# stratosphere/rdfind

Hardware: AMD Instinct MI355X
Metric: CIND-discovery triples/sec (higher is better)
Workload: dtype u32

## Files before the change

rdfind_amd/_lib.py:

```python
from __future__ import annotations

import ctypes
import os

import numpy as np

from . import codes

_HERE = os.path.dirname(os.path.abspath(__file__))
LIB_PATH = os.environ.get("RDFIND_HIP_LIB") or os.path.join(_HERE, "librdfind_hip.so")

RDF_CLEAN_IMPLIED = 1
RDF_STRATEGY_ALL_AT_ONCE = 2
RDF_SHARD_LOCAL_SLICE = 4
RDF_USE_ASSOCIATION_RULES = 8

EXPORTED_SYMBOLS = (
    "rdf_ctx_create", "rdf_ctx_destroy", "rdf_last_error", "rdf_version", "rdf_set_triples",
    "rdf_set_triples_device", "rdf_frequent_conditions", "rdf_build_capture_groups", "rdf_discover_cinds",
    "rdf_run", "rdf_cind_count", "rdf_copy_cinds", "rdf_decode_capture", "rdf_binary_key_count",
    "rdf_copy_binary_keys", "rdf_stage_times", "rdf_kernel_times", "rdf_sync",
    "rdf_copy_cinds_range", "rdf_cind_checksum", "rdf_last_stats", "rdf_shard_begin", "rdf_shard_step",
    "rdf_shard_export", "rdf_shard_import", "rdf_set_dictionary", "rdf_format_size", "rdf_format_cinds",
    "rdf_distinct_triples", "rdf_copy_triples", "rdf_parse_ntriples", "rdf_copy_terms",
# ... 3 lines not shown
    "rdf_discover_cinds_paged", "rdf_next_page", "rdf_shard_parse_begin", "rdf_shard_dictionary_begin", "rdf_num_terms",
    "rdf_dictionary_terms", "rdf_copy_result_refs", "rdf_release_scratch", "rdf_set_handover",
    "rdf_copy_result_refs_async", "rdf_handover_wait", "rdf_set_result_form", "rdf_heavy_chunk_count",
    "rdf_copy_result_heavy", "rdf_parse_begin", "rdf_parse_chunk", "rdf_parse_end", "rdf_copy_term_heap",
    "rdf_rewrite_terms", "rdf_condition_histogram", "rdf_join_histogram", "rdf_copy_histogram", "rdf_count_literals",
    "rdf_cind_stats_begin", "rdf_cind_stats_add", "rdf_cind_stats_end", "rdf_cind_histogram", "rdf_copy_top_refs",
    "rdf_select_cinds", "rdf_selected_count", "rdf_copy_selected_decoded", "rdf_format_selected_size",
    "rdf_format_selected", "rdf_find_terms", "rdf_check_cinds", "rdf_copy_check_rows", "rdf_copy_check_examples",
)
RDF_CHK_ABSENT = 0xFFFFFFFE
RDF_CHK_MAX_EXAMPLES = 16
RDF_SEL_ANY = 0xFFFFFFFF
RDF_SEL_MAX_PATTERNS = 256
RDF_SEL_COUNT_ONLY = 1
SEL_CODES = (10, 12, 14, 17, 20, 21, 33, 34, 35)
SEL_ALL_CODES = 0x1FF
RDF_CS_SHAPE, RDF_CS_SUPPORT, RDF_CS_REFS, RDF_CS_INDEGREE = 1, 2, 3, 4
RDF_JH_NO_FIS = 1
RDF_RW_ASCIIFY = 1
RDF_NT_TABS = 1

TEST_SYMBOLS = ("rdf_test_scan", "rdf_test_scan_batch", "rdf_test_radix", "rdf_test_radix_passes",
                "rdf_test_radix_segments", "rdf_test_paths", "rdf_test_rewrite_form", "rdf_test_cind_stats_times",
                "rdf_test_fc_trace", "rdf_test_fc_report", "rdf_test_copy_frequent_unary", "rdf_test_unary_lookup")
REWRITE_FORMS = {0: None, 1: "lds", 2: "global"}
SCAN_U32_U32, SCAN_U32_U64, SCAN_U64_U64 = range(3)
SCAN_DTYPES = {SCAN_U32_U32: (np.uint32, np.uint32), SCAN_U32_U64: (np.uint32, np.uint64),
               SCAN_U64_U64: (np.uint64, np.uint64)}
RADIX_SORT_BITS, RADIX_SORT_DROP, RADIX_PART_HASHED, RADIX_PART_U32 = range(4)
K1_FORMS = {0: None, 1: "partitioned", 2: "radix", 3: "atomic"}
K2_FORMS = {0: None, 1: "plain", 2: "split", 3: "radix", 4: "atomic"}
K3_FORMS = {0: None, 1: "onepass", 2: "twopass"}

X_DONE, X_ALLREDUCE_SUM_U32, X_ALLREDUCE_SUM_U64, X_ALLREDUCE_MIN_U64, X_ALLGATHERV_U64, X_ALLTOALLV_U64 = range(6)
MAX_RANKS = 64

TIMER_NAMES = ("unary", "binary", "emit", "sort", "support", "groups", "heavymask", "pivot", "light", "esort",
               "hcount", "rules", "hwrite", "class", "cemit")


class FcStats(ctypes.Structure):
    _fields_ = [("min_support", ctypes.c_uint32), ("n_ar_suppressed", ctypes.c_uint32),
                ("n_frequent_unary", ctypes.c_uint64 * 3), ("n_binary_keys", ctypes.c_uint64),
                ("n_frequent_binary", ctypes.c_uint64)]


class ParseStats(ctypes.Structure):
# ... 200 lines not shown
        "rdf_dictionary_terms": (i32, [P, P, u64, P, u64, P]),
        "rdf_discover_cinds_paged": (i32, [P, u32, u64, ctypes.POINTER(CindStats)]),
        "rdf_next_page": (i32, [P, ctypes.POINTER(u32), ctypes.POINTER(u64), ctypes.POINTER(u64)]),
        "rdf_host_free": (None, [P]),
        "rdf_shard_begin": (i32, [P, u32, u32, u32, ctypes.c_char_p, u32]),
        "rdf_shard_step": (i32, [P, ctypes.POINTER(Exchange)]),
        "rdf_shard_export": (i32, [P, P]),
        "rdf_shard_import": (i32, [P, P, u64]),
        "rdf_test_scan": (i32, [P, ctypes.c_int, P, u64, u32, u32, ctypes.c_int, ctypes.c_int, P, ctypes.POINTER(u64),
                                ctypes.POINTER(u32)]),
        "rdf_test_scan_batch": (i32, [P, ctypes.c_int, P, u64, u32, P, ctypes.POINTER(u32)]),
        "rdf_test_radix": (i32, [P, ctypes.c_int, P, u64, ctypes.c_int, ctypes.c_int, u64, P, ctypes.POINTER(u64),
                                 ctypes.POINTER(u32)]),
        "rdf_test_radix_passes": (ctypes.c_int, [ctypes.c_int]),
        "rdf_test_radix_segments": (i32, [P, P, u64, P, u64, P, u32, ctypes.c_int, ctypes.c_int, ctypes.c_int32, u32, u32,
                                          P, ctypes.POINTER(u64), ctypes.POINTER(u32)]),
        "rdf_test_paths": (i32, [P, ctypes.POINTER(PathReport)]),
        "rdf_test_rewrite_form": (i32, [P, ctypes.POINTER(u32)]),
        "rdf_test_cind_stats_times": (i32, [P, ctypes.POINTER(ctypes.c_float)]),
        "rdf_test_fc_trace": (i32, [P, ctypes.c_int]),
        "rdf_test_fc_report": (i32, [P, ctypes.POINTER(FcReport)]),
        "rdf_test_copy_frequent_unary": (i32, [P, P, u64, ctypes.POINTER(u64), ctypes.POINTER(u64)]),
        "rdf_test_unary_lookup": (i32, [P, P, u64, P, P, ctypes.POINTER(u32)]),
    }
    for name, (res, args) in sig.items():
        fn = getattr(lib, name, None) if name in TEST_SYMBOLS else getattr(lib, name)
        if fn is None:
            continue
        fn.restype = res
        fn.argtypes = args
    _lib = lib
    return lib


class PinnedBuffer:

    def __init__(self, count: int, dtype):
        self.lib = load()
        self.nbytes = max(int(count), 1) * np.dtype(dtype).itemsize
        self.ptr = self.lib.rdf_host_alloc(self.nbytes)
        if not self.ptr:
            raise RdfError(f"rdf_host_alloc({self.nbytes}) failed")
        self.array = np.ctypeslib.as_array((ctypes.c_uint8 * self.nbytes).from_address(self.ptr)).view(dtype)

    def __del__(self):
        if getattr(self, "ptr", None):
# ... 414 lines not shown
        out = np.empty_like(a)
        n_out, ok = ctypes.c_uint64(), ctypes.c_uint32()
        rc = self._test_fn("rdf_test_radix")(self.ptr, op, a.ctypes.data, a.shape[0], lo, hi, hmask, out.ctypes.data,
                                     ctypes.byref(n_out), ctypes.byref(ok))
        self.test_canaries_ok = bool(ok.value)
        self._check(rc, "rdf_test_radix")
        return out[: n_out.value], bool(ok.value)

    def test_radix_segments(self, src, counts, bases=None, stride=0, w0=0, bits=64, bump=None):
        a = np.ascontiguousarray(src, dtype=np.uint64)
        cnt = np.ascontiguousarray(counts, dtype=np.uint64)
        base = None if bases is None else np.ascontiguousarray(bases, dtype=np.uint64)
        assert base is None or base.shape == cnt.shape
        out = np.empty(max(int(cnt.sum()), 1), np.uint64)
        bseg, bdig, bdelta = bump if bump else (0, 0, 0)
        n_out, ok = ctypes.c_uint64(), ctypes.c_uint32()
        rc = self._test_fn("rdf_test_radix_segments")(
            self.ptr, a.ctypes.data, a.shape[0], None if base is None else base.ctypes.data, stride, cnt.ctypes.data,
            cnt.shape[0], w0, bits, bdelta, bseg, bdig, out.ctypes.data, ctypes.byref(n_out), ctypes.byref(ok))
        self.test_canaries_ok = bool(ok.value)
        self._check(rc, "rdf_test_radix_segments")
        return out[: n_out.value], bool(ok.value)

    def test_paths(self) -> dict:
        r = PathReport()
        self._check(self._test_fn("rdf_test_paths")(self.ptr, ctypes.byref(r)), "rdf_test_paths")
        d = _struct_dict(r)
        d["k1_form"], d["k2_form"], d["k3_form"] = K1_FORMS[r.k1_form], K2_FORMS[r.k2_form], K3_FORMS[r.k3_form]
        for name in ("dense_on", "light_stage", "light_hiocc", "light_ordered", "light_side", "light_two_pass", "sig_on",
                     "piv2_on", "k3_hist"):
            d[name] = bool(d[name])
        return d

    def test_fc_trace(self, on: bool = True):
        self._check(self._test_fn("rdf_test_fc_trace")(self.ptr, int(on)), "rdf_test_fc_trace")

    def test_fc_report(self) -> dict:
        r = FcReport()
        self._check(self._test_fn("rdf_test_fc_report")(self.ptr, ctypes.byref(r)), "rdf_test_fc_report")
        d = _struct_dict(r)
        d["k1_form"], d["k2_form"], d["traced"] = K1_FORMS[r.k1_form], K2_FORMS[r.k2_form], bool(r.traced)
        return d

    def test_copy_frequent_unary(self):
        U, n3 = ctypes.c_uint64(), (ctypes.c_uint64 * 3)()
        fn = self._test_fn("rdf_test_copy_frequent_unary")
# ... 257 lines not shown
```

rdfind_amd/csrc/rdfind_hip.hip:

```cpp
#include <algorithm>
#include <cstdio>
#include <cstring>
#include <cstdlib>
#include <string>
#include <chrono>
#include <vector>
#include <utility>
#include <initializer_list>
#include <unordered_map>

#include "../../include/rdfind_hip.h"
#include "test_abi.h"
#include "primitives.hpp"
#include "radix_host.hpp"
#include "kernels.inl"
#include "switches.hpp"

using namespace rdf;

#define RDF_VERSION "rdfind_amd 0.1 (gfx950)"

#define RDF_CTX_BUFFERS(B) \
     \
    B(INPUT, scal) \
// ... 38 lines not shown
     \
     \
     \
     \
     \
    B(RUN, chk_rows) B(RUN, chk_ex) B(RUN, chk_cand) B(RUN, chk_keys) B(RUN, chk_keys_tmp) B(RUN, chk_flag) B(RUN, chk_pos) \
    B(RUN, chk_ucap) B(RUN, chk_side) B(RUN, chk_cnt) B(RUN, chk_inb) B(RUN, chk_tab) B(RUN, chk_w) B(RUN, chk_woff) \
    B(RUN, chk_rec) B(RUN, chk_rec_tmp) B(RUN, chk_qval) B(RUN, chk_qoff) B(RUN, chk_nit) B(RUN, chk_ioff) \
    B(RUN, chk_viol) B(RUN, chk_vpre) B(RUN, chk_scal) \
     \
    B(RUN, frank) B(RUN, fval) B(RUN, fext) \
    B(RUN, cnt) B(SPARE_FC, tkeys) B(RUN, tcnt) B(RUN, bkeys) B(RUN, bkeys_tmp) B(RUN, lkeys) B(RUN, lvals) B(RUN, flags) \
    B(RUN, pos) \
     \
    B(RUN, uhist) B(SPARE_FC, urecs) B(RUN, usl) B(RUN, cntg) B(RUN, fstage) B(RUN, bfreq) B(RUN, boff) B(RUN, fbits) \
    B(SPARE_FC, brkeys) \
     \
    B(SPARE_FC, brkeys2) B(RUN, bstart2) \
     \
     \
    B(RUN, arcnt) B(RUN, ar_bits) B(RUN, ar_rules) B(RUN, arref) \
     \
    B(SPARE_GROUPS, rec) B(SPARE_GROUPS, rec_tmp) B(RUN, support) B(RUN, fidx) B(RUN, fcap) B(RUN, info) \
    B(SPARE_GROUPS, fk) B(SPARE_GROUPS, fk_tmp) B(RUN, fpos) B(RUN, cstart) B(RUN, skip) B(RUN, gflag) B(RUN, gexcl) \
    B(RUN, goff) B(RUN, gcap) B(RUN, gmap) B(RUN, csup) B(RUN, doff) B(RUN, dcur) B(RUN, dgrp) \
    B(RUN, hist) B(RUN, heavy_list) B(RUN, hbit) B(RUN, bcomp) B(RUN, bkeyc) B(RUN, pcnt) B(RUN, poff) B(RUN, pcur) \
    B(RUN, plist) \
     \
     \
    B(RUN, jhist) B(RUN, rsup) B(RUN, offp) B(RUN, jbh) B(RUN, lsup) \
     \
     \
     \
    B(SPARE_GROUPS, rstore) B(RUN, jrmap) B(RUN, ecache) \
     \
    B(RUN, ukey) B(RUN, utab) B(RUN, urep) B(RUN, ucnt) B(RUN, unoff) B(RUN, uebin) B(RUN, umem) \
     \
    B(RUN, hot) B(RUN, hotc) \
     \
    B(RUN, pivot) B(RUN, nchl) B(RUN, nchh) B(RUN, choffl) B(RUN, choffh) B(RUN, epairs) B(RUN, epairs_tmp) B(RUN, eoff) \
    B(RUN, hcounts) B(RUN, hoff) B(RUN, hbits) B(RUN, cbits) B(RUN, hown) B(RUN, cown) B(RUN, sbase) B(RUN, dcls) \
    B(RUN, crep) B(RUN, out) B(RUN, stage_rows) \
     \
    B(INPUT, dheap) B(INPUT, dtoff) B(RUN, cslen) B(RUN, csoff) B(RUN, cstr) B(RUN, flen) B(RUN, floff) B(RUN, fbuf) \
     \
    B(RUN, drows) B(RUN, ppart) \
     \
// ... 1974 lines not shown
    tend(c, RDF_T_EMIT);
    u64 Je = 0;
    if (n && !onepass) {
        TRY(read_u64(c, overflow, &c->hscal[8]));
        if (c->hscal[8])
            return fail(c, RDF_ERR_LIMIT, "K3: a block emitted more records than its scanned region (records past it "
                                          "were not written)");
    }
    if (reuse) {
        Je = c->ecache_je[slot];
    } else {
        if (je_early == ~0ull) {
            TRY(read_scalars(c, onepass ? 4 : 1));
            je_early = c->hscal[0];
            if (onepass && n && c->hscal[3] >= je_early) c->J_emit += c->hscal[3] - je_early;
        }
        Je = je_early;
        if (cache > 0) c->ecache_je[slot] = Je;
    }
    if (Je > slot_cap) return fail(c, RDF_ERR_LIMIT, "K3 emitted more records than the join range was sized for");
    return g_sort_support(c, ebuf, c->rec_tmp.as<u64>(), Je, sup, Jout, nullptr);
}

static rdf_status g_fresh_bounds(rdf_ctx* c, const u64* keys, u64 J) {
    hipStream_t st = c->stream;
    HIP_TRY(c, hipMemsetAsync(c->cstart.p, 0xff, (c->ncap + 1) * 4, st));
    hipLaunchKernelGGL(k_fresh_bounds, dim3(grid_for(J + 1, RDF_BLOCK, kGrid)), dim3(RDF_BLOCK), 0, st, keys, J, c->ncap,
                       c->joinbits, c->flags.as<u32>(), c->cstart.as<u32>());
    hipLaunchKernelGGL(k_cstart_fix, dim3(grid_for(c->ncap + 1, RDF_BLOCK, kGrid)), dim3(RDF_BLOCK), 0, st, keys, J, c->ncap,
                       c->joinbits, c->cstart.as<u32>());
    return RDF_OK;
}

static rdf_status g_sort_support(rdf_ctx* c, u64* keys, u64* tmp, u64 Je, u32* sup, u64* Jout, u64* keep_out) {
    hipStream_t st = c->stream;
    const int capbits = c->capbits, joinbits = c->joinbits;
    c->J_emit += Je;
    u64 J = 0;
    tbegin(c, RDF_T_SORT);
    HIP_TRY(c, radix_sort_u64_drop(c->ws, keys, tmp, Je, capbits + joinbits, (u32*)dscal(c, 1), &J, st));
    if (keep_out && keys != keep_out) {
        if (J) HIP_TRY(c, hipMemcpyAsync(keep_out, keys, J * 8, hipMemcpyDeviceToDevice, st));
        keys = keep_out;
    }
    tend(c, RDF_T_SORT);
    c->sort_passes_records += Je + (u64)(radix_sort_passes(capbits + joinbits) - 1) * J;
    return g_support_sorted(c, keys, J, sup, Jout);
}

static rdf_status g_support_sorted(rdf_ctx* c, u64* keys, u64 J, u32* sup, u64* Jout) {
    hipStream_t st = c->stream;
    const u64 ncap = c->ncap;
    *Jout = J;
    c->rec_sorted = keys;
    ENSURE(c, flags, std::max<u64>(J, 1) * 4);
    ENSURE(c, fpos, (J + 1) * 4);
    ENSURE(c, cstart, (ncap + 1) * 4);
    tbegin(c, RDF_T_SUPPORT);
    TRY(g_fresh_bounds(c, keys, J));
    HIP_TRY(c, exclusive_scan_u32(c->ws, c->flags.as<u32>(), c->fpos.as<u32>(), J, c->fpos.as<u32>() + J, st));
    if (ncap)
        hipLaunchKernelGGL(k_run_support, dim3(grid_for(ncap, RDF_BLOCK, kGrid)), dim3(RDF_BLOCK), 0, st, c->cstart.as<u32>(),
                           ncap, c->fpos.as<u32>(), sup);
    tend(c, RDF_T_SUPPORT);
    return RDF_OK;
}

static rdf_status g_emit_sort_support(rdf_ctx* c, int proj) {
    TRY(g_record_bits(c));
    HIP_TRY(c, hipEventRecord(c->ev[2], c->stream));
    c->J_emit = 0;
    c->sort_passes_records = 0;
    ENSURE(c, support, std::max<u64>(c->ncap, 1) * 4);
    u64 J = 0;
    TRY(g_emit_range(c, proj, shard_sel(c), 9 * c->n, c->support.as<u32>(), &J));
    c->J = J;
    return RDF_OK;
}

static rdf_status g_compact_captures(rdf_ctx* c) {
    hipStream_t st = c->stream;
    const u32 V = c->V ? c->V : 1;
    const u64 ncap = c->ncap;
    ENSURE(c, flags, std::max<u64>(ncap, 1) * 4);
    ENSURE(c, fidx, (ncap + 1) * 4);
    hipLaunchKernelGGL(k_support_flags, dim3(grid_for(ncap, RDF_BLOCK, kGrid)), dim3(RDF_BLOCK), 0, st,
                       c->support.as<u32>(), ncap, c->ms, c->flags.as<u32>());
    HIP_TRY(c, exclusive_scan_u32(c->ws, c->flags.as<u32>(), c->fidx.as<u32>(), ncap, c->fidx.as<u32>() + ncap, st));
    u32 C = 0, Cu = 0;
    {
        u64 v[2];
        TRY(read_multi(c, {{c->fidx.as<u32>() + ncap, 4}, {c->fidx.as<u32>() + 2ull * c->U, 4}}, v));
        C = (u32)v[0];
        Cu = (u32)v[1];
    }
    c->C = C;
    c->Cu = Cu;
    ENSURE(c, fcap, std::max<u64>(C, 1) * 4);
    ENSURE(c, info, std::max<u64>(C, 1) * sizeof(CapInfo));
    hipLaunchKernelGGL(k_compact_captures, dim3(grid_for(ncap, RDF_BLOCK, kGrid)), dim3(RDF_BLOCK), 0, st,
                       c->support.as<u32>(), c->fidx.as<u32>(), ncap, c->ms, c->fcap.as<u32>(), c->info.as<CapInfo>());
    ENSURE(c, fext, std::max<u64>(C, 1) * 4);
    if (C)
        hipLaunchKernelGGL(k_external_ids, dim3(grid_for(C, RDF_BLOCK, kGrid)), dim3(RDF_BLOCK), 0, st, c->fcap.as<u32>(), C,
                           2u * c->U, V, c->fval.as<u32>(), c->Us, c->Up, c->fext.as<u32>());
    return RDF_OK;
}

static rdf_status g_compact_groups(rdf_ctx* c) {
    hipStream_t st = c->stream;
    const u32 V = c->V ? c->V : 1;
    const u64 ncap = c->ncap, J = c->J;
    const int joinbits = c->joinbits;
    u64* keys = c->rec_sorted;
    tbegin(c, RDF_T_SUPPORT);
    ENSURE(c, flags, std::max(J, ncap) * 4);
    TRY(g_compact_captures(c));
    const u32 C = c->C;
    ENSURE(c, skip, (ncap + 1) * 4);
    if (ncap)
        hipLaunchKernelGGL(k_skip_counts, dim3(grid_for(ncap, RDF_BLOCK, kGrid)), dim3(RDF_BLOCK), 0, st, c->cstart.as<u32>(),
                           c->fpos.as<u32>(), c->support.as<u32>(), ncap, c->ms, c->flags.as<u32>());
    HIP_TRY(c, exclusive_scan_u32(c->ws, c->flags.as<u32>(), c->skip.as<u32>(), ncap, c->skip.as<u32>() + ncap, st));
    u64 fs[2];
    TRY(read_multi(c, {{c->fpos.as<u32>() + J, 4}, {c->skip.as<u32>() + ncap, 4}}, fs));
    const u64 Jf = fs[0] - fs[1];
    c->Jf = Jf;
    u64* dk = keys == c->rec.as<u64>() ? c->rec_tmp.as<u64>() : c->rec.as<u64>();
    ENSURE(c, fk, std::max<u64>(Jf, 1) * 8);
    ENSURE(c, fk_tmp, std::max<u64>(Jf, 1) * 8);
    if (J)
        hipLaunchKernelGGL(k_keep_scatter, dim3(grid_for(J, RDF_BLOCK, kGrid)), dim3(RDF_BLOCK), 0, st, keys, J, joinbits,
                           c->fpos.as<u32>(), c->skip.as<u32>(), c->support.as<u32>(), c->ms, c->fidx.as<u32>(), dk,
                           c->fk.as<u64>());
    tend(c, RDF_T_SUPPORT);
    tbegin(c, RDF_T_GROUPS);
    ENSURE(c, csup, std::max<u64>(C, 1) * 4);
    ENSURE(c, doff, (C + 1ull) * 8);
    ENSURE(c, dgrp, std::max<u64>(Jf, 1) * 4);
    if (C)
        hipLaunchKernelGGL(k_info_support_u32, dim3(grid_for(C, RDF_BLOCK, kGrid)), dim3(RDF_BLOCK), 0, st,
                           c->info.as<CapInfo>(), C, c->csup.as<u32>());
    if (Jf) {
        hipLaunchKernelGGL(k_key_offsets, dim3(grid_for(C + 1ull, RDF_BLOCK, kGrid)), dim3(RDF_BLOCK), 0, st, dk, Jf, C,
                           c->doff.as<u64>());
        u64* tk = c->fk.as<u64>();
        u64* tt = c->fk_tmp.as<u64>();
        HIP_TRY(c, radix_sort_u64_bits(c->ws, tk, tt, Jf, 32, 32 + joinbits, st));
        if (tk != c->fk.as<u64>()) std::swap(c->fk, c->fk_tmp);
    } else {
        HIP_TRY(c, hipMemsetAsync(c->doff.p, 0, (C + 1ull) * 8, st));
    }
    ENSURE(c, gflag, std::max<u64>(Jf, 1) * 4);
    ENSURE(c, gexcl, (Jf + 1) * 4);
    if (Jf)
        hipLaunchKernelGGL(k_group_flags, dim3(grid_for(Jf, RDF_BLOCK, kGrid)), dim3(RDF_BLOCK), 0, st, c->fk.as<u64>(), Jf,
                           c->gflag.as<u32>());
    HIP_TRY(c, exclusive_scan_u32(c->ws, c->gflag.as<u32>(), c->gexcl.as<u32>(), Jf, c->gexcl.as<u32>() + Jf, st));
    u32 G32 = 0;
    TRY(read_u32(c, c->gexcl.as<u32>() + Jf, &G32));
    const u64 G = G32;
    c->G = G;
    ENSURE(c, goff, (G + 1) * 8);
    ENSURE(c, gcap, std::max<u64>(Jf, 1) * 4 + 16);
    ENSURE(c, gmap, (u64)V * 4);
    if (Jf) {
        hipLaunchKernelGGL(k_group_build, dim3(grid_for(Jf, RDF_BLOCK, kGrid)), dim3(RDF_BLOCK), 0, st, c->fk.as<u64>(), Jf,
                           c->gflag.as<u32>(), c->gexcl.as<u32>(), c->goff.as<u64>(), c->gcap.as<u32>(), c->gmap.as<u32>());
        hipLaunchKernelGGL(k_dgrp, dim3(grid_for(Jf, RDF_BLOCK, kGrid)), dim3(RDF_BLOCK), 0, st, dk, Jf, c->gmap.as<u32>(),
                           c->dgrp.as<u32>());
    }
    c->hscal[14] = Jf;
    HIP_TRY(c, hipMemcpyAsync(c->goff.as<u64>() + G, c->hscal + 14, 8, hipMemcpyHostToDevice, st));
    tend(c, RDF_T_GROUPS);
    return RDF_OK;
}

static rdf_status g_range_keep_plan(rdf_ctx* c) {
    const std::vector<rdf_ctx::JoinRange>& ranges = c->jranges;
    c->jr_keep = false;
    if (!c->sw.range_keep || ranges.empty() || ranges.size() > EMIT_MAX_RANGES) return RDF_OK;
    u64 total = 0;
    c->jr_seg.assign(ranges.size() + 1, 0);
    c->jr_J.assign(ranges.size(), 0);
    for (size_t k = 0; k < ranges.size(); ++k) {
        c->jr_seg[k] = total;
        total += ranges[k].recs;
    }
    c->jr_seg[ranges.size()] = total;
    size_t free_b = 0, total_b = 0;
    if (hipMemGetInfo(&free_b, &total_b) != hipSuccess) return RDF_OK;
// ... 130 lines not shown
    for (size_t k = 0; k < ranges.size(); ++k) {
        const rdf_ctx::JoinRange& r = ranges[k];
        u64 J = 0;
        JoinSel js = own;
        js.lo = r.lo;
        js.hi = r.hi;
        if (c->jr_keep) {
            u64* seg = c->rstore.as<u64>() + c->jr_seg[k];
            TRY(g_sort_support(c, seg, c->rec.as<u64>(), c->jr_seg[k + 1] - c->jr_seg[k], c->rsup.as<u32>(), &J, seg));
            c->jr_J[k] = J;
        } else {
            TRY(g_emit_range(c, proj, js, cap_rec, c->rsup.as<u32>(), &J, 1 + (int)k));
        }
        Jtot += J;
        if (ncap)
            hipLaunchKernelGGL(k_add_u32, dim3(grid_for(ncap, RDF_BLOCK, kGrid)), dim3(RDF_BLOCK), 0, st, c->support.as<u32>(),
                               c->rsup.as<u32>(), ncap);
    }
    c->J = Jtot;
    return RDF_OK;
}

static rdf_status g_restore_range(rdf_ctx* c, size_t k, u64* Jout) {
    hipStream_t st = c->stream;
    const u64 J = c->jr_J[k], ncap = c->ncap;
    u64* keys = c->rstore.as<u64>() + c->jr_seg[k];
    ENSURE(c, flags, std::max<u64>(J, 1) * 4);
    ENSURE(c, fpos, (J + 1) * 4);
    ENSURE(c, cstart, (ncap + 1) * 4);
    ENSURE(c, rec, std::max<u64>(c->jr_cap_rec, 1) * 8);
    tbegin(c, RDF_T_SUPPORT);
    TRY(g_fresh_bounds(c, keys, J));
    HIP_TRY(c, exclusive_scan_u32(c->ws, c->flags.as<u32>(), c->fpos.as<u32>(), J, c->fpos.as<u32>() + J, st));
    tend(c, RDF_T_SUPPORT);
    c->rec_sorted = keys;
    *Jout = J;
    return RDF_OK;
}

static rdf_status g_ranges_groups(rdf_ctx* c, int proj, JoinSel own, const u32* local_sup) {
    hipStream_t st = c->stream;
    const u32 V = c->V ? c->V : 1;
    const u64 ncap = c->ncap;
    const int joinbits = c->joinbits;
    const std::vector<rdf_ctx::JoinRange>& ranges = c->jranges;
    const u64 cap_rec = c->jr_cap_rec;
    const u64 J_emit = c->J_emit, Jtot = c->J;
    tbegin(c, RDF_T_SUPPORT);
    TRY(g_compact_captures(c));
    const u32 C = c->C;
    ENSURE(c, csup, std::max<u64>(C, 1) * 4);
    ENSURE(c, doff, (C + 1ull) * 8);
    ENSURE(c, dcur, std::max<u64>(C, 1) * 4);
    if (C)
        hipLaunchKernelGGL(k_info_support_u32, dim3(grid_for(C, RDF_BLOCK, kGrid)), dim3(RDF_BLOCK), 0, st,
                           c->info.as<CapInfo>(), C, c->csup.as<u32>());
// ... 8 lines not shown
    tend(c, RDF_T_SUPPORT);
    u64 Jf = 0;
    TRY(read_u64(c, c->doff.as<u64>() + C, &Jf));
    c->Jf = Jf;
    const u64 Gmax = std::min<u64>(V, Jf);
    ENSURE(c, goff, (Gmax + 1) * 8);
    ENSURE(c, gcap, std::max<u64>(Jf, 1) * 4 + 16);
    ENSURE(c, gmap, (u64)V * 4);
    ENSURE(c, dgrp, std::max<u64>(Jf, 1) * 4);
    ENSURE(c, offp, (C + 1ull) * 8);
    ENSURE(c, skip, (ncap + 1) * 4);
    HIP_TRY(c, hipMemsetAsync(c->dcur.p, 0, std::max<u64>(C, 1) * 4, st));
    u64 Jf0 = 0, G0 = 0;
    for (size_t k = 0; k < ranges.size(); ++k) {
        const rdf_ctx::JoinRange& r = ranges[k];
        u64 J = 0;
        JoinSel js = own;
        js.lo = r.lo;
        js.hi = r.hi;
        if (c->jr_keep) TRY(g_restore_range(c, k, &J));
        else TRY(g_emit_range(c, proj, js, cap_rec, c->rsup.as<u32>(), &J, -1 - (int)k));
        u64* keys = c->rec_sorted;
        tbegin(c, RDF_T_SUPPORT);
        ENSURE(c, flags, std::max<u64>(std::max<u64>(J, ncap), 1) * 4);
        if (ncap)
            hipLaunchKernelGGL(k_skip_counts, dim3(grid_for(ncap, RDF_BLOCK, kGrid)), dim3(RDF_BLOCK), 0, st, c->cstart.as<u32>(),
                               c->fpos.as<u32>(), c->support.as<u32>(), ncap, c->ms, c->flags.as<u32>());
        HIP_TRY(c, exclusive_scan_u32(c->ws, c->flags.as<u32>(), c->skip.as<u32>(), ncap, c->skip.as<u32>() + ncap, st));
        u64 fs[2];
        TRY(read_multi(c, {{c->fpos.as<u32>() + J, 4}, {c->skip.as<u32>() + ncap, 4}}, fs));
        const u64 Jr = fs[0] - fs[1];
        u64* dk = keys == c->rec.as<u64>() ? c->rec_tmp.as<u64>() : c->rec.as<u64>();
        ENSURE(c, fk, std::max<u64>(Jr, 1) * 8);
        ENSURE(c, fk_tmp, std::max<u64>(Jr, 1) * 8);
        if (J)
            hipLaunchKernelGGL(k_keep_scatter, dim3(grid_for(J, RDF_BLOCK, kGrid)), dim3(RDF_BLOCK), 0, st, keys, J, joinbits,
                               c->fpos.as<u32>(), c->skip.as<u32>(), c->support.as<u32>(), c->ms, c->fidx.as<u32>(), dk,
                               c->fk.as<u64>());
        tend(c, RDF_T_SUPPORT);
        tbegin(c, RDF_T_GROUPS);
        if (Jr) {
            u64* tk = c->fk.as<u64>();
            u64* tt = c->fk_tmp.as<u64>();
            HIP_TRY(c, radix_sort_u64_bits(c->ws, tk, tt, Jr, 32, 32 + joinbits, st));
            if (tk != c->fk.as<u64>()) std::swap(c->fk, c->fk_tmp);
        }
        ENSURE(c, gflag, std::max<u64>(Jr, 1) * 4);
        ENSURE(c, gexcl, (Jr + 1) * 4);
        if (Jr)
            hipLaunchKernelGGL(k_group_flags, dim3(grid_for(Jr, RDF_BLOCK, kGrid)), dim3(RDF_BLOCK), 0, st, c->fk.as<u64>(), Jr,
                               c->gflag.as<u32>());
        HIP_TRY(c, exclusive_scan_u32(c->ws, c->gflag.as<u32>(), c->gexcl.as<u32>(), Jr, c->gexcl.as<u32>() + Jr, st));
        u32 Gr = 0;
        TRY(read_u32(c, c->gexcl.as<u32>() + Jr, &Gr));
        if (G0 + Gr > Gmax || Jf0 + Jr > Jf) return fail(c, RDF_ERR_LIMIT, "join ranges disagree on the kept records");
        if (Jr) {
            hipLaunchKernelGGL(k_group_build_at, dim3(grid_for(Jr, RDF_BLOCK, kGrid)), dim3(RDF_BLOCK), 0, st, c->fk.as<u64>(), Jr,
                               c->gflag.as<u32>(), c->gexcl.as<u32>(), Jf0, (u32)G0, c->goff.as<u64>(), c->gcap.as<u32>(),
                               c->gmap.as<u32>());
            hipLaunchKernelGGL(k_key_offsets, dim3(grid_for(C + 1ull, RDF_BLOCK, kGrid)), dim3(RDF_BLOCK), 0, st, dk, Jr, C,
                               c->offp.as<u64>());
            hipLaunchKernelGGL(k_dgrp_range, dim3(grid_for(Jr, RDF_BLOCK, kGrid)), dim3(RDF_BLOCK), 0, st, dk, Jr,
                               c->offp.as<u64>(), c->doff.as<u64>(), c->dcur.as<u32>(), c->gmap.as<u32>(), c->dgrp.as<u32>());
            if (C)
                hipLaunchKernelGGL(k_dcur_add, dim3(grid_for(C, RDF_BLOCK, kGrid)), dim3(RDF_BLOCK), 0, st, c->offp.as<u64>(), C,
                                   c->dcur.as<u32>());
        }
        tend(c, RDF_T_GROUPS);
        Jf0 += Jr;
        G0 += Gr;
    }
    if (Jf0 != Jf) return fail(c, RDF_ERR_LIMIT, "join ranges disagree on the kept records");
    c->G = G0;
    c->J = Jtot;
    c->J_emit = J_emit;
    c->hscal[14] = Jf;
    HIP_TRY(c, hipMemcpyAsync(c->goff.as<u64>() + G0, c->hscal + 14, 8, hipMemcpyHostToDevice, st));
    HIP_TRY(c, hipStreamSynchronize(st));
    c->rec_sorted = nullptr;
    return RDF_OK;
}

// ... 129 lines not shown
    if (stats) {
        TRY(settle_group_stats(c));
        *stats = c->gstats;
    }
    c->stage = 3;
    return RDF_OK;
}

rdf_status rdf_build_capture_groups(rdf_ctx* c, const char* projection, rdf_group_stats* stats) {
    if (!c) return RDF_ERR_ARG;
    if (c->stage < 2) return fail(c, RDF_ERR_STATE, "rdf_frequent_conditions must be called first");
    HIP_TRY(c, hipSetDevice(c->device));
    TRY(hv_wait(c, true));
    int proj = 0;
    TRY(parse_projection(c, projection, &proj));
    c->rank = 0;
    c->nranks = 1;
    c->paged = c->cs_open = c->cs_top_valid = c->sel_valid = false;
    c->n_group_ranges = 1;
    if (c->sw.group_range_records || 9 * c->n >= (1ull << 32)) {
        TRY(g_build_ranges(c, proj, c->sw.group_range_records ? c->sw.group_range_records : auto_range_records(c)));
    } else {
        TRY(g_emit_sort_support(c, proj));
        TRY(g_compact_groups(c));
    }
    if (c->ar_on) TRY(g_ar_refs(c));
    TRY(g_size_hist(c, nullptr));
    TRY(g_heavy_binary(c, 0, 0, true));
    return g_finish(c, stats);
}


static CindView make_view(rdf_ctx* c, uint32_t flags) {
    CindView v;
    v.C = c->C;
    v.Cu = c->Cu;
    v.info = c->info.as<CapInfo>();
    v.gcap = c->gcap.as<u32>();
    v.goff = c->goff.as<u64>();
    v.hbit = c->hbit.as<uint8_t>();
    v.doff = c->doff.as<u64>();
    v.dgrp = c->dgrp.as<u32>();
    v.bcomp = c->bcomp.as<u32>();
    v.bkeyc = c->bkeyc.as<u64>();
    v.poff = c->poff.as<u64>();
    v.plist = c->plist.as<u32>();
    v.eoff = nullptr;
// ... 1513 lines not shown
    }
};

static rdf_status sh_phase14(rdf_ctx* c, rdf_exchange* req) {
    hipStream_t st = c->stream;
    const u64 m = c->x_recv_count / 2;
    ENSURE(c, wts, std::max<u64>(m, 1) * 4);
    ENSURE(c, wtp, std::max<u64>(m, 1) * 4);
    ENSURE(c, wto, std::max<u64>(m, 1) * 4);
    if (m)
        hipLaunchKernelGGL(k_unpack_triples, dim3(grid_for(m, RDF_BLOCK, kGrid)), dim3(RDF_BLOCK), 0, st, c->xrecv.as<u64>(), m,
                           c->wts.as<u32>(), c->wtp.as<u32>(), c->wto.as<u32>());
    c->spare_x = true;
    c->rank = c->sh_rank;
    c->nranks = c->sh_nranks;
    c->sh_m = m;
    c->sh_ranged = c->sw.group_range_records || 9 * m >= (1ull << 32);
    c->n_group_ranges = 1;
    {
        ReceivedTriples rt(c);
        if (c->sh_ranged) {
            TRY(g_ranges_supports(c, c->sh_proj, c->sw.group_range_records ? c->sw.group_range_records : auto_range_records(c),
                                  shard_sel(c)));
            ENSURE(c, lsup, std::max<u64>(c->ncap, 1) * 4);
            HIP_TRY(c, hipMemcpyAsync(c->lsup.p, c->support.p, std::max<u64>(c->ncap, 1) * 4, hipMemcpyDeviceToDevice, st));
        } else {
            TRY(g_emit_sort_support(c, c->sh_proj));
        }
    }
    HIP_TRY(c, hipStreamSynchronize(st));
    return x_request(c, req, RDF_X_ALLREDUCE_SUM_U32, c->support.p, c->ncap, 1);
}

static rdf_status sh_phase1(rdf_ctx* c, rdf_exchange* req) {
    HIP_TRY(c, hipMemcpyAsync(c->support.p, c->xrecv.p, c->ncap * 4, hipMemcpyDeviceToDevice, c->stream));
    if (c->sh_ranged) {
        ReceivedTriples rt(c);
        TRY(g_ranges_groups(c, c->sh_proj, shard_sel(c), c->lsup.as<u32>()));
    } else {
        TRY(g_compact_groups(c));
    }
    c->spare_x = false;
    if (c->ar_on) TRY(g_ar_refs(c));
    TRY(g_size_hist(c, c->h_hist_local));
    ENSURE(c, xsend, 256 * 8);
    std::vector<u64> w(256);
    for (int i = 0; i < 256; ++i) w[i] = c->h_hist_local[i];
    HIP_TRY(c, ctx_copy(c, c->xsend.p, w.data(), 256 * 8, hipMemcpyHostToDevice));
    return x_request(c, req, RDF_X_ALLGATHERV_U64, c->xsend.p, 256, 2);
}

static rdf_status sh_phase2(rdf_ctx* c, rdf_exchange* req) {
    const u32 R = c->nranks;
    if (c->x_recv_count != 256ull * R) return fail(c, RDF_ERR_ARG, "histogram all-gather: wrong element count");
    std::vector<u64> all(256ull * R);
    HIP_TRY(c, ctx_copy(c, all.data(), c->xrecv.p, all.size() * 8, hipMemcpyDeviceToHost));
    u32 gh[256] = {};
    for (u32 r = 0; r < R; ++r)
        for (int b = 0; b < 256; ++b) gh[b] += (u32)all[256ull * r + b];
    const u64 thr = heavy_threshold(c, gh);
    u32 base = 0;
    for (u32 r = 0; r < c->rank; ++r) {
        u32 lh[256];
// ... 2220 lines not shown
```

Baseline: 1.524 billion.

## Replace per-record flag scans with per-tile counts in support and group build

The support and grouping stages previously wrote a flag per record, scanned the full flag arrays and used separate cstart/fix/run-support kernels. Now k_fresh_bounds counts fresh records per tile and accumulates support directly, and group heads are counted per tile. Only the small tile-count arrays are scanned, and the keep-scatter and group-build kernels use the tile bases. This removes full-length scans and intermediate arrays, in exchange for in-kernel tile-local scans and a new local-support path for sharding. It also adds test hooks.

```diff
diff --git a/rdfind_amd/_lib.py b/rdfind_amd/_lib.py
--- a/rdfind_amd/_lib.py
+++ b/rdfind_amd/_lib.py
@@ -49,7 +49,8 @@
 
 TEST_SYMBOLS = ("rdf_test_scan", "rdf_test_scan_batch", "rdf_test_radix", "rdf_test_radix_passes",
                 "rdf_test_radix_segments", "rdf_test_paths", "rdf_test_rewrite_form", "rdf_test_cind_stats_times",
-                "rdf_test_fc_trace", "rdf_test_fc_report", "rdf_test_copy_frequent_unary", "rdf_test_unary_lookup")
+                "rdf_test_fc_trace", "rdf_test_fc_report", "rdf_test_copy_frequent_unary", "rdf_test_unary_lookup",
+                "rdf_test_record_tile", "rdf_test_keep_records", "rdf_test_group_build")
 REWRITE_FORMS = {0: None, 1: "lds", 2: "global"}
 SCAN_U32_U32, SCAN_U32_U64, SCAN_U64_U64 = range(3)
 SCAN_DTYPES = {SCAN_U32_U32: (np.uint32, np.uint32), SCAN_U32_U64: (np.uint32, np.uint64),
@@ -296,6 +297,10 @@
         "rdf_test_fc_report": (i32, [P, ctypes.POINTER(FcReport)]),
         "rdf_test_copy_frequent_unary": (i32, [P, P, u64, ctypes.POINTER(u64), ctypes.POINTER(u64)]),
         "rdf_test_unary_lookup": (i32, [P, P, u64, P, P, ctypes.POINTER(u32)]),
+        "rdf_test_record_tile": (ctypes.c_int, []),
+        "rdf_test_keep_records": (i32, [P, P, u64, ctypes.c_int, u64, u32, P, ctypes.POINTER(u64), ctypes.POINTER(u32), P, P,
+                                        P, ctypes.POINTER(u32)]),
+        "rdf_test_group_build": (i32, [P, P, u64, u32, u64, u32, ctypes.POINTER(u64), P, P, P, ctypes.POINTER(u32)]),
     }
     for name, (res, args) in sig.items():
         fn = getattr(lib, name, None) if name in TEST_SYMBOLS else getattr(lib, name)
@@ -756,6 +761,35 @@
         self._check(rc, "rdf_test_radix_segments")
         return out[: n_out.value], bool(ok.value)
 
+    def test_record_tile(self) -> int:
+        return int(self._test_fn("rdf_test_record_tile")())
+
+    def test_keep_records(self, keys, joinbits: int, ncap: int, ms: int):
+        a = np.ascontiguousarray(keys, dtype=np.uint64)
+        sup = np.empty(ncap, np.uint32)
+        dk, fk = np.empty(max(a.shape[0], 1), np.uint64), np.empty(max(a.shape[0], 1), np.uint64)
+        doff = np.empty(ncap + 1, np.uint64)
+        jf, ncomp, ok = ctypes.c_uint64(), ctypes.c_uint32(), ctypes.c_uint32()
+        rc = self._test_fn("rdf_test_keep_records")(
+            self.ptr, a.ctypes.data, a.shape[0], joinbits, ncap, ms, sup.ctypes.data, ctypes.byref(jf), ctypes.byref(ncomp),
+            dk.ctypes.data, fk.ctypes.data, doff.ctypes.data, ctypes.byref(ok))
+        self.test_canaries_ok = bool(ok.value)
+        self._check(rc, "rdf_test_keep_records")
+        return sup, dk[: jf.value], fk[: jf.value], doff[: ncomp.value + 1], bool(ok.value)
+
+    def test_group_build(self, fk, num_values: int, rbase=0, gbase=0):
+        a = np.ascontiguousarray(fk, dtype=np.uint64)
+        goff = np.empty(a.shape[0] + 1, np.uint64)
+        gcap = np.empty(max(a.shape[0], 1), np.uint32)
+        gmap = np.empty(num_values, np.uint32)
+        g, ok = ctypes.c_uint64(), ctypes.c_uint32()
+        rc = self._test_fn("rdf_test_group_build")(
+            self.ptr, a.ctypes.data, a.shape[0], num_values, rbase, gbase, ctypes.byref(g), goff.ctypes.data,
+            gcap.ctypes.data, gmap.ctypes.data, ctypes.byref(ok))
+        self.test_canaries_ok = bool(ok.value)
+        self._check(rc, "rdf_test_group_build")
+        return goff[: g.value + 1], gcap[: a.shape[0]], gmap, bool(ok.value)
+
     def test_paths(self) -> dict:
         r = PathReport()
         self._check(self._test_fn("rdf_test_paths")(self.ptr, ctypes.byref(r)), "rdf_test_paths")
diff --git a/rdfind_amd/csrc/rdfind_hip.hip b/rdfind_amd/csrc/rdfind_hip.hip
--- a/rdfind_amd/csrc/rdfind_hip.hip
+++ b/rdfind_amd/csrc/rdfind_hip.hip
@@ -84,7 +84,11 @@
     B(RUN, arcnt) B(RUN, ar_bits) B(RUN, ar_rules) B(RUN, arref) \
      \
     B(SPARE_GROUPS, rec) B(SPARE_GROUPS, rec_tmp) B(RUN, support) B(RUN, fidx) B(RUN, fcap) B(RUN, info) \
-    B(SPARE_GROUPS, fk) B(SPARE_GROUPS, fk_tmp) B(RUN, fpos) B(RUN, cstart) B(RUN, skip) B(RUN, gflag) B(RUN, gexcl) \
+     \
+     \
+     \
+    B(SPARE_GROUPS, fk) B(SPARE_GROUPS, fk_tmp) B(RUN, tile_fresh) B(RUN, tile_base) B(RUN, tile_heads) B(RUN, tile_gbase) \
+    B(RUN, skip) B(RUN, fpos) B(RUN, gflag) B(RUN, gexcl) \
     B(RUN, goff) B(RUN, gcap) B(RUN, gmap) B(RUN, csup) B(RUN, doff) B(RUN, dcur) B(RUN, dgrp) \
     B(RUN, hist) B(RUN, heavy_list) B(RUN, hbit) B(RUN, bcomp) B(RUN, bkeyc) B(RUN, pcnt) B(RUN, poff) B(RUN, pcur) \
     B(RUN, plist) \
@@ -2105,13 +2109,17 @@
     return g_sort_support(c, ebuf, c->rec_tmp.as<u64>(), Je, sup, Jout, nullptr);
 }
 
-static rdf_status g_fresh_bounds(rdf_ctx* c, const u64* keys, u64 J) {
-    hipStream_t st = c->stream;
-    HIP_TRY(c, hipMemsetAsync(c->cstart.p, 0xff, (c->ncap + 1) * 4, st));
-    hipLaunchKernelGGL(k_fresh_bounds, dim3(grid_for(J + 1, RDF_BLOCK, kGrid)), dim3(RDF_BLOCK), 0, st, keys, J, c->ncap,
-                       c->joinbits, c->flags.as<u32>(), c->cstart.as<u32>());
-    hipLaunchKernelGGL(k_cstart_fix, dim3(grid_for(c->ncap + 1, RDF_BLOCK, kGrid)), dim3(RDF_BLOCK), 0, st, keys, J, c->ncap,
-                       c->joinbits, c->cstart.as<u32>());
+static inline unsigned rec_tiles(u64 n) { return (unsigned)((n + KT_TILE - 1) / KT_TILE); }
+
+static rdf_status g_fresh_bounds(rdf_ctx* c, const u64* keys, u64 J, u32* sup) {
+    hipStream_t st = c->stream;
+    const unsigned nt = rec_tiles(J);
+    ENSURE(c, tile_fresh, std::max<u64>(nt, 1) * 4);
+    ENSURE(c, tile_base, (nt + 1ull) * 4);
+    HIP_TRY(c, hipMemsetAsync(sup, 0, std::max<u64>(c->ncap, 1) * 4, st));
+    if (nt)
+        hipLaunchKernelGGL(k_fresh_bounds, dim3(nt), dim3(RDF_BLOCK), 0, st, keys, J, c->joinbits, c->tile_fresh.as<u32>(), sup);
+    HIP_TRY(c, exclusive_scan_u32(c->ws, c->tile_fresh.as<u32>(), c->tile_base.as<u32>(), nt, c->tile_base.as<u32>() + nt, st));
     return RDF_OK;
 }
 
@@ -2132,19 +2140,10 @@
 }
 
 static rdf_status g_support_sorted(rdf_ctx* c, u64* keys, u64 J, u32* sup, u64* Jout) {
-    hipStream_t st = c->stream;
-    const u64 ncap = c->ncap;
     *Jout = J;
     c->rec_sorted = keys;
-    ENSURE(c, flags, std::max<u64>(J, 1) * 4);
-    ENSURE(c, fpos, (J + 1) * 4);
-    ENSURE(c, cstart, (ncap + 1) * 4);
     tbegin(c, RDF_T_SUPPORT);
-    TRY(g_fresh_bounds(c, keys, J));
-    HIP_TRY(c, exclusive_scan_u32(c->ws, c->flags.as<u32>(), c->fpos.as<u32>(), J, c->fpos.as<u32>() + J, st));
-    if (ncap)
-        hipLaunchKernelGGL(k_run_support, dim3(grid_for(ncap, RDF_BLOCK, kGrid)), dim3(RDF_BLOCK), 0, st, c->cstart.as<u32>(),
-                           ncap, c->fpos.as<u32>(), sup);
+    TRY(g_fresh_bounds(c, keys, J, sup));
     tend(c, RDF_T_SUPPORT);
     return RDF_OK;
 }
@@ -2190,32 +2189,41 @@
     return RDF_OK;
 }
 
-static rdf_status g_compact_groups(rdf_ctx* c) {
+static rdf_status g_group_heads(rdf_ctx* c, u64 Jr, u32* Gout) {
+    hipStream_t st = c->stream;
+    const unsigned nt = rec_tiles(Jr);
+    ENSURE(c, tile_heads, std::max<u64>(nt, 1) * 4);
+    ENSURE(c, tile_gbase, (nt + 1ull) * 4);
+    if (nt) hipLaunchKernelGGL(k_group_flags, dim3(nt), dim3(RDF_BLOCK), 0, st, c->fk.as<u64>(), Jr, c->tile_heads.as<u32>());
+    HIP_TRY(c, exclusive_scan_u32(c->ws, c->tile_heads.as<u32>(), c->tile_gbase.as<u32>(), nt, c->tile_gbase.as<u32>() + nt, st));
+    return read_u32(c, c->tile_gbase.as<u32>() + nt, Gout);
+}
+
+static rdf_status g_compact_groups(rdf_ctx* c, const u32* local_sup) {
     hipStream_t st = c->stream;
     const u32 V = c->V ? c->V : 1;
     const u64 ncap = c->ncap, J = c->J;
     const int joinbits = c->joinbits;
     u64* keys = c->rec_sorted;
     tbegin(c, RDF_T_SUPPORT);
-    ENSURE(c, flags, std::max(J, ncap) * 4);
     TRY(g_compact_captures(c));
     const u32 C = c->C;
     ENSURE(c, skip, (ncap + 1) * 4);
     if (ncap)
-        hipLaunchKernelGGL(k_skip_counts, dim3(grid_for(ncap, RDF_BLOCK, kGrid)), dim3(RDF_BLOCK), 0, st, c->cstart.as<u32>(),
-                           c->fpos.as<u32>(), c->support.as<u32>(), ncap, c->ms, c->flags.as<u32>());
+        hipLaunchKernelGGL(k_skip_counts, dim3(grid_for(ncap, RDF_BLOCK, kGrid)), dim3(RDF_BLOCK), 0, st,
+                           local_sup ? local_sup : c->support.as<u32>(), c->support.as<u32>(), ncap, c->ms, c->flags.as<u32>());
     HIP_TRY(c, exclusive_scan_u32(c->ws, c->flags.as<u32>(), c->skip.as<u32>(), ncap, c->skip.as<u32>() + ncap, st));
+    const unsigned nt = rec_tiles(J);
     u64 fs[2];
-    TRY(read_multi(c, {{c->fpos.as<u32>() + J, 4}, {c->skip.as<u32>() + ncap, 4}}, fs));
+    TRY(read_multi(c, {{c->tile_base.as<u32>() + nt, 4}, {c->skip.as<u32>() + ncap, 4}}, fs));
     const u64 Jf = fs[0] - fs[1];
     c->Jf = Jf;
     u64* dk = keys == c->rec.as<u64>() ? c->rec_tmp.as<u64>() : c->rec.as<u64>();
     ENSURE(c, fk, std::max<u64>(Jf, 1) * 8);
     ENSURE(c, fk_tmp, std::max<u64>(Jf, 1) * 8);
-    if (J)
-        hipLaunchKernelGGL(k_keep_scatter, dim3(grid_for(J, RDF_BLOCK, kGrid)), dim3(RDF_BLOCK), 0, st, keys, J, joinbits,
-                           c->fpos.as<u32>(), c->skip.as<u32>(), c->support.as<u32>(), c->ms, c->fidx.as<u32>(), dk,
-                           c->fk.as<u64>());
+    if (nt)
+        hipLaunchKernelGGL(k_keep_scatter, dim3(nt), dim3(RDF_BLOCK), 0, st, keys, J, joinbits, c->tile_base.as<u32>(),
+                           c->skip.as<u32>(), c->support.as<u32>(), c->ms, c->fidx.as<u32>(), dk, c->fk.as<u64>());
     tend(c, RDF_T_SUPPORT);
     tbegin(c, RDF_T_GROUPS);
     ENSURE(c, csup, std::max<u64>(C, 1) * 4);
@@ -2224,32 +2232,31 @@
     if (C)
         hipLaunchKernelGGL(k_info_support_u32, dim3(grid_for(C, RDF_BLOCK, kGrid)), dim3(RDF_BLOCK), 0, st,
                            c->info.as<CapInfo>(), C, c->csup.as<u32>());
+    const u32* nrec = c->csup.as<u32>();
+    if (local_sup) {
+        ENSURE(c, dcur, std::max<u64>(C, 1) * 4);
+        if (C)
+            hipLaunchKernelGGL(k_gather_u32, dim3(grid_for(C, RDF_BLOCK, kGrid)), dim3(RDF_BLOCK), 0, st, local_sup,
+                               c->fcap.as<u32>(), (u64)C, c->dcur.as<u32>());
+        nrec = c->dcur.as<u32>();
+    }
+    HIP_TRY(c, exclusive_scan_u32_u64(c->ws, nrec, c->doff.as<u64>(), C, c->doff.as<u64>() + C, st));
     if (Jf) {
-        hipLaunchKernelGGL(k_key_offsets, dim3(grid_for(C + 1ull, RDF_BLOCK, kGrid)), dim3(RDF_BLOCK), 0, st, dk, Jf, C,
-                           c->doff.as<u64>());
         u64* tk = c->fk.as<u64>();
         u64* tt = c->fk_tmp.as<u64>();
         HIP_TRY(c, radix_sort_u64_bits(c->ws, tk, tt, Jf, 32, 32 + joinbits, st));
         if (tk != c->fk.as<u64>()) std::swap(c->fk, c->fk_tmp);
-    } else {
-        HIP_TRY(c, hipMemsetAsync(c->doff.p, 0, (C + 1ull) * 8, st));
-    }
-    ENSURE(c, gflag, std::max<u64>(Jf, 1) * 4);
-    ENSURE(c, gexcl, (Jf + 1) * 4);
-    if (Jf)
-        hipLaunchKernelGGL(k_group_flags, dim3(grid_for(Jf, RDF_BLOCK, kGrid)), dim3(RDF_BLOCK), 0, st, c->fk.as<u64>(), Jf,
-                           c->gflag.as<u32>());
-    HIP_TRY(c, exclusive_scan_u32(c->ws, c->gflag.as<u32>(), c->gexcl.as<u32>(), Jf, c->gexcl.as<u32>() + Jf, st));
+    }
     u32 G32 = 0;
-    TRY(read_u32(c, c->gexcl.as<u32>() + Jf, &G32));
+    TRY(g_group_heads(c, Jf, &G32));
     const u64 G = G32;
     c->G = G;
     ENSURE(c, goff, (G + 1) * 8);
     ENSURE(c, gcap, std::max<u64>(Jf, 1) * 4 + 16);
     ENSURE(c, gmap, (u64)V * 4);
     if (Jf) {
-        hipLaunchKernelGGL(k_group_build, dim3(grid_for(Jf, RDF_BLOCK, kGrid)), dim3(RDF_BLOCK), 0, st, c->fk.as<u64>(), Jf,
-                           c->gflag.as<u32>(), c->gexcl.as<u32>(), c->goff.as<u64>(), c->gcap.as<u32>(), c->gmap.as<u32>());
+        hipLaunchKernelGGL(k_group_build, dim3(rec_tiles(Jf)), dim3(RDF_BLOCK), 0, st, c->fk.as<u64>(), Jf,
+                           c->tile_gbase.as<u32>(), c->goff.as<u64>(), c->gcap.as<u32>(), c->gmap.as<u32>());
         hipLaunchKernelGGL(k_dgrp, dim3(grid_for(Jf, RDF_BLOCK, kGrid)), dim3(RDF_BLOCK), 0, st, dk, Jf, c->gmap.as<u32>(),
                            c->dgrp.as<u32>());
     }
@@ -2426,16 +2433,11 @@
 }
 
 static rdf_status g_restore_range(rdf_ctx* c, size_t k, u64* Jout) {
-    hipStream_t st = c->stream;
-    const u64 J = c->jr_J[k], ncap = c->ncap;
+    const u64 J = c->jr_J[k];
     u64* keys = c->rstore.as<u64>() + c->jr_seg[k];
-    ENSURE(c, flags, std::max<u64>(J, 1) * 4);
-    ENSURE(c, fpos, (J + 1) * 4);
-    ENSURE(c, cstart, (ncap + 1) * 4);
     ENSURE(c, rec, std::max<u64>(c->jr_cap_rec, 1) * 8);
     tbegin(c, RDF_T_SUPPORT);
-    TRY(g_fresh_bounds(c, keys, J));
-    HIP_TRY(c, exclusive_scan_u32(c->ws, c->flags.as<u32>(), c->fpos.as<u32>(), J, c->fpos.as<u32>() + J, st));
+    TRY(g_fresh_bounds(c, keys, J, c->rsup.as<u32>()));
     tend(c, RDF_T_SUPPORT);
     c->rec_sorted = keys;
     *Jout = J;
@@ -2490,21 +2492,21 @@
         else TRY(g_emit_range(c, proj, js, cap_rec, c->rsup.as<u32>(), &J, -1 - (int)k));
         u64* keys = c->rec_sorted;
         tbegin(c, RDF_T_SUPPORT);
-        ENSURE(c, flags, std::max<u64>(std::max<u64>(J, ncap), 1) * 4);
+        ENSURE(c, flags, std::max<u64>(ncap, 1) * 4);
         if (ncap)
-            hipLaunchKernelGGL(k_skip_counts, dim3(grid_for(ncap, RDF_BLOCK, kGrid)), dim3(RDF_BLOCK), 0, st, c->cstart.as<u32>(),
-                               c->fpos.as<u32>(), c->support.as<u32>(), ncap, c->ms, c->flags.as<u32>());
+            hipLaunchKernelGGL(k_skip_counts, dim3(grid_for(ncap, RDF_BLOCK, kGrid)), dim3(RDF_BLOCK), 0, st, c->rsup.as<u32>(),
+                               c->support.as<u32>(), ncap, c->ms, c->flags.as<u32>());
         HIP_TRY(c, exclusive_scan_u32(c->ws, c->flags.as<u32>(), c->skip.as<u32>(), ncap, c->skip.as<u32>() + ncap, st));
+        const unsigned nt = rec_tiles(J);
         u64 fs[2];
-        TRY(read_multi(c, {{c->fpos.as<u32>() + J, 4}, {c->skip.as<u32>() + ncap, 4}}, fs));
+        TRY(read_multi(c, {{c->tile_base.as<u32>() + nt, 4}, {c->skip.as<u32>() + ncap, 4}}, fs));
         const u64 Jr = fs[0] - fs[1];
         u64* dk = keys == c->rec.as<u64>() ? c->rec_tmp.as<u64>() : c->rec.as<u64>();
         ENSURE(c, fk, std::max<u64>(Jr, 1) * 8);
         ENSURE(c, fk_tmp, std::max<u64>(Jr, 1) * 8);
-        if (J)
-            hipLaunchKernelGGL(k_keep_scatter, dim3(grid_for(J, RDF_BLOCK, kGrid)), dim3(RDF_BLOCK), 0, st, keys, J, joinbits,
-                               c->fpos.as<u32>(), c->skip.as<u32>(), c->support.as<u32>(), c->ms, c->fidx.as<u32>(), dk,
-                               c->fk.as<u64>());
+        if (nt)
+            hipLaunchKernelGGL(k_keep_scatter, dim3(nt), dim3(RDF_BLOCK), 0, st, keys, J, joinbits, c->tile_base.as<u32>(),
+                               c->skip.as<u32>(), c->support.as<u32>(), c->ms, c->fidx.as<u32>(), dk, c->fk.as<u64>());
         tend(c, RDF_T_SUPPORT);
         tbegin(c, RDF_T_GROUPS);
         if (Jr) {
@@ -2513,19 +2515,12 @@
             HIP_TRY(c, radix_sort_u64_bits(c->ws, tk, tt, Jr, 32, 32 + joinbits, st));
             if (tk != c->fk.as<u64>()) std::swap(c->fk, c->fk_tmp);
         }
-        ENSURE(c, gflag, std::max<u64>(Jr, 1) * 4);
-        ENSURE(c, gexcl, (Jr + 1) * 4);
-        if (Jr)
-            hipLaunchKernelGGL(k_group_flags, dim3(grid_for(Jr, RDF_BLOCK, kGrid)), dim3(RDF_BLOCK), 0, st, c->fk.as<u64>(), Jr,
-                               c->gflag.as<u32>());
-        HIP_TRY(c, exclusive_scan_u32(c->ws, c->gflag.as<u32>(), c->gexcl.as<u32>(), Jr, c->gexcl.as<u32>() + Jr, st));
         u32 Gr = 0;
-        TRY(read_u32(c, c->gexcl.as<u32>() + Jr, &Gr));
+        TRY(g_group_heads(c, Jr, &Gr));
         if (G0 + Gr > Gmax || Jf0 + Jr > Jf) return fail(c, RDF_ERR_LIMIT, "join ranges disagree on the kept records");
         if (Jr) {
-            hipLaunchKernelGGL(k_group_build_at, dim3(grid_for(Jr, RDF_BLOCK, kGrid)), dim3(RDF_BLOCK), 0, st, c->fk.as<u64>(), Jr,
-                               c->gflag.as<u32>(), c->gexcl.as<u32>(), Jf0, (u32)G0, c->goff.as<u64>(), c->gcap.as<u32>(),
-                               c->gmap.as<u32>());
+            hipLaunchKernelGGL(k_group_build_at, dim3(rec_tiles(Jr)), dim3(RDF_BLOCK), 0, st, c->fk.as<u64>(), Jr,
+                               c->tile_gbase.as<u32>(), Jf0, (u32)G0, c->goff.as<u64>(), c->gcap.as<u32>(), c->gmap.as<u32>());
             hipLaunchKernelGGL(k_key_offsets, dim3(grid_for(C + 1ull, RDF_BLOCK, kGrid)), dim3(RDF_BLOCK), 0, st, dk, Jr, C,
                                c->offp.as<u64>());
             hipLaunchKernelGGL(k_dgrp_range, dim3(grid_for(Jr, RDF_BLOCK, kGrid)), dim3(RDF_BLOCK), 0, st, dk, Jr,
@@ -2701,7 +2696,7 @@
         TRY(g_build_ranges(c, proj, c->sw.group_range_records ? c->sw.group_range_records : auto_range_records(c)));
     } else {
         TRY(g_emit_sort_support(c, proj));
-        TRY(g_compact_groups(c));
+        TRY(g_compact_groups(c, nullptr));
     }
     if (c->ar_on) TRY(g_ar_refs(c));
     TRY(g_size_hist(c, nullptr));
@@ -4261,11 +4256,11 @@
         if (c->sh_ranged) {
             TRY(g_ranges_supports(c, c->sh_proj, c->sw.group_range_records ? c->sw.group_range_records : auto_range_records(c),
                                   shard_sel(c)));
-            ENSURE(c, lsup, std::max<u64>(c->ncap, 1) * 4);
-            HIP_TRY(c, hipMemcpyAsync(c->lsup.p, c->support.p, std::max<u64>(c->ncap, 1) * 4, hipMemcpyDeviceToDevice, st));
         } else {
             TRY(g_emit_sort_support(c, c->sh_proj));
         }
+        ENSURE(c, lsup, std::max<u64>(c->ncap, 1) * 4);
+        HIP_TRY(c, hipMemcpyAsync(c->lsup.p, c->support.p, std::max<u64>(c->ncap, 1) * 4, hipMemcpyDeviceToDevice, st));
     }
     HIP_TRY(c, hipStreamSynchronize(st));
     return x_request(c, req, RDF_X_ALLREDUCE_SUM_U32, c->support.p, c->ncap, 1);
@@ -4277,7 +4272,7 @@
         ReceivedTriples rt(c);
         TRY(g_ranges_groups(c, c->sh_proj, shard_sel(c), c->lsup.as<u32>()));
     } else {
-        TRY(g_compact_groups(c));
+        TRY(g_compact_groups(c, c->lsup.as<u32>()));
     }
     c->spare_x = false;
     if (c->ar_on) TRY(g_ar_refs(c));
```

Result: faster. 1.612 billion, median of 6 (+5.8%).
